# rostin79s/TFHE-AES

Hardware: AMD Instinct MI355X
Metric: AES-128 CTR blocks/sec (FHE) (higher is better)
Workload: dtype u64+f64; 1 GPU; configs[2]: 128 CTR blocks per GPU, Server::aes_encrypt 10 rounds (1280 bit-CBS/block), counters pre-incremented client-side; params=PARAM_OPT, blocks_per_gpu=128, total_blocks=128

## Files before the change

### tfhe_aes_amd/csrc/kern_keyswitch.h

```cpp
#pragma once
#include <hip/hip_runtime.h>
#include <stdint.h>
#include "fft_dev.h"

#define KS_CT_TILE 64
#define KS_KSTEP 64

typedef int ks_int4 __attribute__((ext_vector_type(4)));

struct KeyswitchArgs {
    const int8_t *afrag;
    const int8_t *bfrag;
    uint32_t ksteps, coltiles;
    const uint64_t *in;
    uint64_t in_stride;
    int32_t body_index;
    uint32_t body_col;
    uint32_t ncols;
    uint64_t *out;
    uint64_t out_stride, out_z_stride;
    uint64_t m;
};

#define KSL_CT_TILES 8
#define KSL_THREADS (64 * KSL_CT_TILES)
#define KSL_COL_TILES 4

#ifndef FHEAES_KS_DECLS_ONLY
__global__ __launch_bounds__(256) void keybytes_kernel(const uint64_t *key, uint64_t key_z_stride, uint32_t rows, uint32_t ncols,
                                                       uint32_t ksteps, uint32_t coltiles, int8_t *frag)
{
    const uint64_t gid = (uint64_t)blockIdx.x * blockDim.x + threadIdx.x;
    const uint32_t lane = gid & 63;
    const uint64_t t = gid >> 6;
    const uint32_t C = t % coltiles;
    const uint32_t ks = (uint32_t)(t / coltiles);
    const uint32_t z = blockIdx.y;
    if (ks >= ksteps) return;
    const uint32_t col = C * 16 + (lane & 15);
    const uint32_t row0 = ks * KS_KSTEP + (lane >> 4) * 16;
    int8_t b[8][16];
#pragma unroll
    for (int e = 0; e < 16; ++e) {
        uint64_t x = 0;
        if (col < ncols && row0 + e < rows) x = key[(uint64_t)z * key_z_stride + (uint64_t)(row0 + e) * ncols + col];
        uint32_t carry = 0;
#pragma unroll
        for (int j = 0; j < 8; ++j) {
            uint32_t v = (uint32_t)((x >> (8 * j)) & 0xFF) + carry;
            carry = v >= 128 ? 1u : 0u;
            b[j][e] = (int8_t)(v & 0xFF);
        }
    }
    int8_t *o = frag + ((((uint64_t)z * ksteps + ks) * coltiles + C) * 8) * 1024 + (uint64_t)lane * 16;
#pragma unroll
    for (int j = 0; j < 8; ++j) {
        ks_int4 w;
        memcpy(&w, b[j], 16);
        *reinterpret_cast<ks_int4 *>(o + (uint64_t)j * 1024) = w;
    }
}

template <int BASE_LOG, int LEVELS, int PLANES>
__global__ __launch_bounds__(256) void digits_kernel(const uint64_t *in, uint64_t in_stride, uint32_t n_in, uint64_t m,
                                                     uint32_t ksteps, int8_t *frag)
{
    const uint64_t gid = (uint64_t)blockIdx.x * blockDim.x + threadIdx.x;
    const uint32_t lane = gid & 63;
    const uint64_t t = gid >> 6;
    const uint32_t ks = t % ksteps;
    const uint64_t T = t / ksteps;
    const uint64_t ct = T * 16 + (lane & 15);
    const uint32_t q0 = ks * KS_KSTEP + (lane >> 4) * 16;
    int8_t lo[16], hi[16];
#pragma unroll
    for (int e = 0; e < 16; ++e) { lo[e] = 0; hi[e] = 0; }
    if (ct < m) {
        const uint32_t i0 = q0 / LEVELS;
        constexpr int NI = (16 + LEVELS - 1) / LEVELS + 1;
#pragma unroll
        for (int ii = 0; ii < NI; ++ii) {
            const uint32_t i = i0 + ii;
            if (i >= n_in) break;
            int d[LEVELS];
            decompose_all<BASE_LOG, LEVELS>(in[ct * in_stride + i], d);
#pragma unroll
            for (int l = 0; l < LEVELS; ++l) {
                const int e = (int)(i * LEVELS + l) - (int)q0;
                if (e >= 0 && e < 16) {
                    const int dl = ((d[l] + 128) & 255) - 128;
#pragma unroll
                    for (int ee = 0; ee < 16; ++ee) if (ee == e) { lo[ee] = (int8_t)dl; hi[ee] = (int8_t)((d[l] - dl) >> 8); }
                }
            }
        }
    }
    int8_t *o = frag + ((T * ksteps + ks) * PLANES) * 1024 + (uint64_t)lane * 16;
    ks_int4 w;
    memcpy(&w, lo, 16);
    *reinterpret_cast<ks_int4 *>(o) = w;
    if (PLANES == 2) {
        memcpy(&w, hi, 16);
        *reinterpret_cast<ks_int4 *>(o + 1024) = w;
    }
}

template <int PLANES>
__global__ __launch_bounds__(KSL_THREADS, 2) void keyswitch_mfma_lds_kernel(const KeyswitchArgs A)
{
    constexpr int A_FRAGS = KSL_CT_TILES * PLANES;
    constexpr int B_FRAGS = KSL_COL_TILES * 8;
    constexpr int FRAGS = A_FRAGS + B_FRAGS;
    __shared__ __attribute__((aligned(16))) int8_t lds[2 * FRAGS * 1024];
    const int lane = threadIdx.x & 63, wave = threadIdx.x >> 6;
    const int wc = wave & 3, wt = wave >> 2;
    const uint32_t C0 = blockIdx.x * KSL_COL_TILES;
    const uint64_t T0 = (uint64_t)blockIdx.y * KSL_CT_TILES;
    const uint32_t z = blockIdx.z;
    const uint64_t ct_tiles_total = (A.m + 15) / 16;

    ks_int4 acc[4][8];
#pragma unroll
    for (int t = 0; t < 4; ++t)
#pragma unroll
        for (int s = 0; s < 8; ++s) acc[t][s] = (ks_int4){0, 0, 0, 0};

    auto issue = [&](uint32_t ks, int buf) {
        constexpr int WAVES = KSL_THREADS / 64;
#pragma unroll
        for (int i = 0; i < (FRAGS + WAVES - 1) / WAVES; ++i) {
            const int f = wave + WAVES * i;
            if (f < FRAGS) {
                const int8_t *src;
                if (f < A_FRAGS) {
                    uint64_t T = T0 + f / PLANES;
                    if (T >= ct_tiles_total) T = ct_tiles_total - 1;
                    src = A.afrag + ((T * A.ksteps + ks) * PLANES + (f % PLANES)) * 1024;
                } else {
                    const int g = f - A_FRAGS;
                    uint32_t C = C0 + g / 8;
                    if (C >= A.coltiles) C = A.coltiles - 1;
                    src = A.bfrag + ((((uint64_t)z * A.ksteps + ks) * A.coltiles + C) * 8 + (g % 8)) * 1024;
                }
                __builtin_amdgcn_global_load_lds((const __attribute__((address_space(1))) void *)(src + lane * 16),
                                                 (__attribute__((address_space(3))) void *)(lds + ((size_t)buf * FRAGS + f) * 1024), 16, 0, 0);
            }
        }
    };

    issue(0, 0);
    for (uint32_t ks = 0; ks < A.ksteps; ++ks) {
        const int buf = ks & 1;
        asm volatile("s_waitcnt vmcnt(0)" ::: "memory");
        __syncthreads();
        if (ks + 1 < A.ksteps) issue(ks + 1, buf ^ 1);
        const int8_t *base = lds + (size_t)buf * FRAGS * 1024 + lane * 16;
        ks_int4 a[4][PLANES], b[8];
#pragma unroll
        for (int s = 0; s < 8; ++s) b[s] = *reinterpret_cast<const ks_int4 *>(base + (A_FRAGS + wc * 8 + s) * 1024);
#pragma unroll
        for (int t = 0; t < 4; ++t)
#pragma unroll
            for (int pl = 0; pl < PLANES; ++pl) a[t][pl] = *reinterpret_cast<const ks_int4 *>(base + ((wt * 4 + t) * PLANES + pl) * 1024);
#pragma unroll
        for (int s = 0; s < 8; ++s) {
#pragma unroll
            for (int t = 0; t < 4; ++t) acc[t][s] = __builtin_amdgcn_mfma_i32_16x16x64_i8(a[t][0], b[s], acc[t][s], 0, 0, 0);
            if (PLANES == 2 && s >= 1) {
#pragma unroll
                for (int t = 0; t < 4; ++t) acc[t][s] = __builtin_amdgcn_mfma_i32_16x16x64_i8(a[t][1], b[s - 1], acc[t][s], 0, 0, 0);
            }
        }
    }

    const uint32_t C = C0 + wc;
    const uint32_t col = C * 16 + (lane & 15);
    if (C >= A.coltiles || col >= A.ncols) return;
#pragma unroll
    for (int t = 0; t < 4; ++t)
#pragma unroll
        for (int r = 0; r < 4; ++r) {
            const uint64_t ct = (T0 + wt * 4 + t) * 16 + (uint64_t)(lane >> 4) * 4 + r;
            if (ct >= A.m) continue;
            uint64_t v = 0;
#pragma unroll
            for (int s = 0; s < 8; ++s) v += (uint64_t)(int64_t)acc[t][s][r] << (8 * s);
            v = (uint64_t)0 - v;
            if (A.body_index >= 0 && col == A.body_col) v += A.in[ct * A.in_stride + (uint32_t)A.body_index];
            A.out[ct * A.out_stride + (uint64_t)z * A.out_z_stride + col] = v;
        }
}
#endif
```

Measured before the change: 61.18 blocks/s.

## Triple-buffer keyswitch MFMA LDS ring with register prefetch of next step's fragments

The LDS staging in the int8 MFMA keyswitch kernel grows from two buffers to a three-deep ring. Global→LDS copies are issued two k-steps ahead through inline-asm global_load_lds with per-wave source pointers that are precomputed once and advanced each step. The A fragments and the first B fragments for the next k-step are read from LDS into registers while the current step's MFMAs run, and sched_barriers keep that interleaving in place. The aim is to hide global-load and LDS-read latency behind MFMA work. In exchange the kernel uses more LDS and more registers, and the hand-written m0/asm sequencing is fragile.

```diff
diff --git a/tfhe_aes_amd/csrc/kern_keyswitch.h b/tfhe_aes_amd/csrc/kern_keyswitch.h
--- a/tfhe_aes_amd/csrc/kern_keyswitch.h
+++ b/tfhe_aes_amd/csrc/kern_keyswitch.h
@@ -25,6 +25,7 @@
 #define KSL_CT_TILES 8
 #define KSL_THREADS (64 * KSL_CT_TILES)
 #define KSL_COL_TILES 4
+#define KSL_RING 3
 
 #ifndef FHEAES_KS_DECLS_ONLY
 __global__ __launch_bounds__(256) void keybytes_kernel(const uint64_t *key, uint64_t key_z_stride, uint32_t rows, uint32_t ncols,
@@ -111,8 +112,9 @@
     constexpr int A_FRAGS = KSL_CT_TILES * PLANES;
     constexpr int B_FRAGS = KSL_COL_TILES * 8;
     constexpr int FRAGS = A_FRAGS + B_FRAGS;
-    __shared__ __attribute__((aligned(16))) int8_t lds[2 * FRAGS * 1024];
-    const int lane = threadIdx.x & 63, wave = threadIdx.x >> 6;
+    constexpr uint32_t BUF = FRAGS * 1024;
+    __shared__ __attribute__((aligned(16))) int8_t lds[KSL_RING * BUF];
+    const int lane = threadIdx.x & 63, wave = __builtin_amdgcn_readfirstlane(threadIdx.x >> 6);
     const int wc = wave & 3, wt = wave >> 2;
     const uint32_t C0 = blockIdx.x * KSL_COL_TILES;
     const uint64_t T0 = (uint64_t)blockIdx.y * KSL_CT_TILES;
@@ -125,53 +127,84 @@
 #pragma unroll
         for (int s = 0; s < 8; ++s) acc[t][s] = (ks_int4){0, 0, 0, 0};
 
-    auto issue = [&](uint32_t ks, int buf) {
-        constexpr int WAVES = KSL_THREADS / 64;
-#pragma unroll
-        for (int i = 0; i < (FRAGS + WAVES - 1) / WAVES; ++i) {
-            const int f = wave + WAVES * i;
-            if (f < FRAGS) {
-                const int8_t *src;
-                if (f < A_FRAGS) {
-                    uint64_t T = T0 + f / PLANES;
-                    if (T >= ct_tiles_total) T = ct_tiles_total - 1;
-                    src = A.afrag + ((T * A.ksteps + ks) * PLANES + (f % PLANES)) * 1024;
-                } else {
-                    const int g = f - A_FRAGS;
-                    uint32_t C = C0 + g / 8;
-                    if (C >= A.coltiles) C = A.coltiles - 1;
-                    src = A.bfrag + ((((uint64_t)z * A.ksteps + ks) * A.coltiles + C) * 8 + (g % 8)) * 1024;
-                }
-                __builtin_amdgcn_global_load_lds((const __attribute__((address_space(1))) void *)(src + lane * 16),
-                                                 (__attribute__((address_space(3))) void *)(lds + ((size_t)buf * FRAGS + f) * 1024), 16, 0, 0);
+    constexpr int WAVES = KSL_THREADS / 64;
+    constexpr int DMAS = FRAGS / WAVES;
+    static_assert(FRAGS % WAVES == 0 && A_FRAGS % WAVES == 0, "every wave issues the same count of each kind");
+    const int8_t *src[DMAS];
+#pragma unroll
+    for (int i = 0; i < DMAS; ++i) {
+        const int f = wave + WAVES * i;
+        if (i < A_FRAGS / WAVES) {
+            uint64_t T = T0 + f / PLANES;
+            if (T >= ct_tiles_total) T = ct_tiles_total - 1;
+            src[i] = A.afrag + (T * A.ksteps * PLANES + (f % PLANES)) * 1024;
+        } else {
+            const int g = f - A_FRAGS;
+            uint32_t C = C0 + g / 8;
+            if (C >= A.coltiles) C = A.coltiles - 1;
+            src[i] = A.bfrag + (((uint64_t)z * A.ksteps * A.coltiles + C) * 8 + (g % 8)) * 1024;
+        }
+    }
+    const uint64_t b_stride = (uint64_t)A.coltiles * 8 * 1024;
+    const uint32_t lds0 = (uint32_t)(uintptr_t)(__attribute__((address_space(3))) int8_t *)lds + wave * 1024, lane16 = lane * 16;
+    auto issue = [&](uint32_t buf) {
+#pragma unroll
+        for (int i = 0; i < DMAS; ++i) {
+            uint32_t keep;
+            asm volatile("s_mov_b32 %0, m0\n\ts_mov_b32 m0, %3\n\ts_nop 0\n\tglobal_load_lds_dwordx4 %1, %2\n\ts_mov_b32 m0, %0"
+                         : "=&s"(keep) : "v"(lane16), "s"(src[i]), "s"(lds0 + buf + WAVES * 1024 * i) : "memory");
+            src[i] += i < A_FRAGS / WAVES ? (uint64_t)PLANES * 1024 : b_stride;
+        }
+    };
+    auto ldb = [&](uint32_t buf, int s) { return *reinterpret_cast<const ks_int4 *>(lds + buf + lane * 16 + (A_FRAGS + wc * 8 + s) * 1024); };
+    auto lda = [&](uint32_t buf, int t, int pl) { return *reinterpret_cast<const ks_int4 *>(lds + buf + lane * 16 + ((wt * 4 + t) * PLANES + pl) * 1024); };
+
+    struct Head { ks_int4 a[4][PLANES], b0, b1; };
+    constexpr int HEAD = 2 + 4 * PLANES;
+    auto ldhead = [&](Head &h, uint32_t buf, int q) {
+        if (q == 0) h.b0 = ldb(buf, 0);
+        else if (q == 5) h.b1 = ldb(buf, 1);
+        else if (q < 5) h.a[q - 1][0] = lda(buf, q - 1, 0);
+        else if (q < HEAD) h.a[q - 6][PLANES - 1] = lda(buf, q - 6, PLANES - 1);
+    };
+
+    uint32_t cur = 0, nxt = BUF, dma = 2 * BUF;
+    auto step = [&](uint32_t ks, const Head &h, Head &hn) {
+        asm volatile("s_waitcnt vmcnt(0)" ::: "memory");
+        __builtin_amdgcn_s_barrier();
+        asm volatile("" ::: "memory");
+        if (ks + 2 < A.ksteps) issue(dma);
+        ks_int4 b[8];
+        b[0] = h.b0; b[1] = h.b1;
+#pragma unroll
+        for (int s = 0; s < 8; ++s) {
+            if (s + 2 < 8) b[s + 2] = ldb(cur, s + 2);
+            if (s >= 2) { ldhead(hn, nxt, 2 * (s - 2)); ldhead(hn, nxt, 2 * (s - 2) + 1); }
+#pragma unroll
+            for (int t = 0; t < 4; ++t) acc[t][s] = __builtin_amdgcn_mfma_i32_16x16x64_i8(h.a[t][0], b[s], acc[t][s], 0, 0, 0);
+            if (PLANES == 2 && s >= 1) {
+#pragma unroll
+                for (int t = 0; t < 4; ++t) acc[t][s] = __builtin_amdgcn_mfma_i32_16x16x64_i8(h.a[t][PLANES - 1], b[s - 1], acc[t][s], 0, 0, 0);
             }
-        }
+            __builtin_amdgcn_sched_barrier(0);
+        }
+        const uint32_t t = cur; cur = nxt; nxt = dma; dma = t;
     };
 
-    issue(0, 0);
-    for (uint32_t ks = 0; ks < A.ksteps; ++ks) {
-        const int buf = ks & 1;
-        asm volatile("s_waitcnt vmcnt(0)" ::: "memory");
-        __syncthreads();
-        if (ks + 1 < A.ksteps) issue(ks + 1, buf ^ 1);
-        const int8_t *base = lds + (size_t)buf * FRAGS * 1024 + lane * 16;
-        ks_int4 a[4][PLANES], b[8];
-#pragma unroll
-        for (int s = 0; s < 8; ++s) b[s] = *reinterpret_cast<const ks_int4 *>(base + (A_FRAGS + wc * 8 + s) * 1024);
-#pragma unroll
-        for (int t = 0; t < 4; ++t)
-#pragma unroll
-            for (int pl = 0; pl < PLANES; ++pl) a[t][pl] = *reinterpret_cast<const ks_int4 *>(base + ((wt * 4 + t) * PLANES + pl) * 1024);
-#pragma unroll
-        for (int s = 0; s < 8; ++s) {
-#pragma unroll
-            for (int t = 0; t < 4; ++t) acc[t][s] = __builtin_amdgcn_mfma_i32_16x16x64_i8(a[t][0], b[s], acc[t][s], 0, 0, 0);
-            if (PLANES == 2 && s >= 1) {
-#pragma unroll
-                for (int t = 0; t < 4; ++t) acc[t][s] = __builtin_amdgcn_mfma_i32_16x16x64_i8(a[t][1], b[s - 1], acc[t][s], 0, 0, 0);
-            }
-        }
-    }
+    Head h0, h1;
+    issue(cur);
+    if (A.ksteps > 1) issue(nxt);
+    asm volatile("s_waitcnt vmcnt(0)" ::: "memory");
+    __builtin_amdgcn_s_barrier();
+    asm volatile("" ::: "memory");
+#pragma unroll
+    for (int q = 0; q < HEAD; ++q) ldhead(h0, cur, q);
+    uint32_t ks = 0;
+    for (; ks + 1 < A.ksteps; ks += 2) {
+        step(ks, h0, h1);
+        step(ks + 1, h1, h0);
+    }
+    if (ks < A.ksteps) step(ks, h0, h1);
 
     const uint32_t C = C0 + wc;
     const uint32_t col = C * 16 + (lane & 15);
```

Result: no change. 61.50 blocks/s (median of 6 runs) (+0.5%).
